# sanderslab/magellanmapper

Measured on AMD Instinct MI355X. Metric: Mvoxels/s, 2048x2048x1024 uint16 stack, 5-sigma LoG blob detection, higher is better.
Workload: dtype f16x2 MFMA (f32 accumulate) + 16-bit fixed-point intermediates; f64 re-score of every candidate

## Files before the change

magellanmapper_amd/csrc/mmx_peaks.hip:

```cpp

#include "mmx_common.h"

namespace {

constexpr int kSigmaChunk = 8;

struct peak_ctx {
    const float* base;
    int64_t sigma_stride;
    int ns, nz, ny, nx, px, plane, slot;
    float thr, eps;
    mmx_cand* out;
    uint32_t cap;
    uint32_t* count;
};

__device__ __forceinline__ void check_voxel(const peak_ctx& c, int s, int idx, float v)
{
    const int z = idx / c.plane;
    const int rem = idx - z * c.plane;
    const int y = rem / c.px;
    const int x = rem - y * c.px;
    const int nz = c.nz, ny = c.ny, nx = c.nx, px = c.px, plane = c.plane;
    const float reject = v + c.eps;
    float m = -INFINITY;
    bool border = false;
    const float* ps = c.base + (int64_t)s * c.sigma_stride;
    if (x > 0) m = fmaxf(m, ps[idx - 1]); else border = true;
    if (x + 1 < nx) m = fmaxf(m, ps[idx + 1]); else border = true;
    if (y > 0) m = fmaxf(m, ps[idx - px]); else border = true;
    if (y + 1 < ny) m = fmaxf(m, ps[idx + px]); else border = true;
    if (z > 0) m = fmaxf(m, ps[idx - plane]); else border = true;
    if (z + 1 < nz) m = fmaxf(m, ps[idx + plane]); else border = true;
    if (m > reject) return;
    for (int ds = -1; ds <= 1; ++ds) {
        const int ss = s + ds;
        if (ss < 0 || ss >= c.ns) { border = true; continue; }
        const float* pss = c.base + (int64_t)ss * c.sigma_stride;
        for (int dz = -1; dz <= 1; ++dz) {
            const int zz = z + dz;
            if (zz < 0 || zz >= nz) continue;
            for (int dy = -1; dy <= 1; ++dy) {
                const int yy = y + dy;
                if (yy < 0 || yy >= ny) continue;
                const int row = zz * plane + yy * px;
#pragma unroll
                for (int dx = -1; dx <= 1; ++dx) {
                    const int xx = x + dx;
                    if (xx < 0 || xx >= nx) continue;
                    if ((ds | dz | dy | dx) == 0) continue;
                    m = fmaxf(m, pss[row + xx]);
                }
            }
            if (m > reject) return;
        }
    }
    if (border) m = fmaxf(m, 0.0f);
    if (!(v >= m - c.eps)) return;
    const bool contested = !(v > m + c.eps) || !(v > c.thr + c.eps);
    const uint32_t pos = atomicAdd(c.count, 1u);
    if (pos < c.cap) {
        mmx_cand r;
        r.slot = c.slot;
        r.s = s;
        r.z = z;
        r.y = y;
        r.x = x;
        r.flags = contested ? MMX_CAND_CONTESTED : 0u;
        r.v = v;
        r.nbr_max = m;
        r.v64 = __longlong_as_double(0x7ff8000000000000LL);
        r.band = 0;
        c.out[pos] = r;
    }
}

__global__ void __launch_bounds__(MMX_WG)
peaks_kernel(const float* __restrict__ log, int ns, int64_t sigma_stride,
             const mmx_block* __restrict__ blocks, int64_t slot_elems, float thr, float eps,
             mmx_cand* __restrict__ out, uint32_t cap, uint32_t* __restrict__ count)
{
    const mmx_block bd = blocks[blockIdx.y];
    peak_ctx c;
    c.base = log + (int64_t)bd.slot * slot_elems;
    c.sigma_stride = sigma_stride;
    c.ns = ns; c.nz = bd.nz; c.ny = bd.ny; c.nx = bd.nx; c.px = bd.px;
    c.plane = bd.ny * bd.px; c.slot = bd.slot;
    c.thr = thr; c.eps = eps; c.out = out; c.cap = cap; c.count = count;
    const int nquads = bd.nz * c.plane / 4;
    const float lo = thr - eps;
    const int qrow = bd.px / 4;

    for (int q = blockIdx.x * MMX_WG + threadIdx.x; q < nquads; q += gridDim.x * MMX_WG) {
        const int x0 = (q % qrow) * 4;
        if (x0 >= bd.nx) continue;
        const float4* p = reinterpret_cast<const float4*>(c.base) + q;
        const int64_t sstride4 = sigma_stride / 4;
        const int lane = threadIdx.x & 63;
        const bool has_left = x0 > 0 && lane > 0;
        const bool has_right = x0 + 4 < bd.nx && lane < 63 && q + 1 < nquads;
        const bool ok1 = x0 + 1 < bd.nx, ok2 = x0 + 2 < bd.nx, ok3 = x0 + 3 < bd.nx;
        for (int s0 = 0; s0 < ns; s0 += kSigmaChunk) {
            float e0[kSigmaChunk + 2], e1[kSigmaChunk + 2], e2[kSigmaChunk + 2], e3[kSigmaChunk + 2];
#pragma unroll
            for (int k = 0; k < kSigmaChunk + 2; ++k) {
                const int s = s0 + k - 1;
                float4 v = make_float4(-INFINITY, -INFINITY, -INFINITY, -INFINITY);
                if (s >= 0 && s < ns) v = p[(int64_t)s * sstride4];
                e0[k] = v.x;
                e1[k] = ok1 ? v.y : -INFINITY;
                e2[k] = ok2 ? v.z : -INFINITY;
                e3[k] = ok3 ? v.w : -INFINITY;
            }
            unsigned hits = 0;
#pragma unroll
            for (int k = 1; k <= kSigmaChunk; ++k) {
                if (s0 + k - 1 < ns) {
                    float lft = __shfl_up(e3[k], 1);
                    float rgt = __shfl_down(e0[k], 1);
                    lft = has_left ? lft : -INFINITY;
                    rgt = has_right ? rgt : -INFINITY;
                    const float n0 = fmaxf(fmaxf(lft, e1[k]), fmaxf(e0[k - 1], e0[k + 1]));
                    const float n1 = fmaxf(fmaxf(e0[k], e2[k]), fmaxf(e1[k - 1], e1[k + 1]));
                    const float n2 = fmaxf(fmaxf(e1[k], e3[k]), fmaxf(e2[k - 1], e2[k + 1]));
                    const float n3 = fmaxf(fmaxf(e2[k], rgt), fmaxf(e3[k - 1], e3[k + 1]));
                    const unsigned sh = 4 * (k - 1);
                    hits |= (mmx_candidate(true, e0[k], lo, eps, n0) ? 1u : 0u) << sh;
                    hits |= (mmx_candidate(true, e1[k], lo, eps, n1) ? 2u : 0u) << sh;
                    hits |= (mmx_candidate(true, e2[k], lo, eps, n2) ? 4u : 0u) << sh;
                    hits |= (mmx_candidate(true, e3[k], lo, eps, n3) ? 8u : 0u) << sh;
                }
            }
            while (hits) {
                const int b = __ffs(hits) - 1;
                hits &= hits - 1;
                const int j = b & 3;
                if (x0 + j >= bd.nx) continue;
                const int s = s0 + (b >> 2);
                const int idx = 4 * q + j;
                check_voxel(c, s, idx, c.base[(int64_t)s * sigma_stride + idx]);
            }
        }
    }
}

struct sparse_ctx {
    peak_ctx c;
    const ulonglong2* ent;
    int64_t ent_sigma_stride;
    mmx_entry_geom eg;
};

__device__ __forceinline__ int64_t sparse_entry(const sparse_ctx& k, int z, int y, int x)
{
    return (int64_t)y * k.eg.per_row + mmx_entry_index(k.eg, z, x);
}

__device__ __forceinline__ float sparse_at(const sparse_ctx& k, int s, int z, int y, int x)
{
    const unsigned long long above = k.ent[(int64_t)s * k.ent_sigma_stride + sparse_entry(k, z, y, x)].y;
    if (!above) return -INFINITY;
    return k.c.base[(int64_t)s * k.c.sigma_stride + (int64_t)z * k.c.plane + y * k.c.px + x];
}

__device__ __forceinline__ void check_voxel_sparse(const sparse_ctx& k, int s, int z, int y, int x, float v)
{
    const peak_ctx& c = k.c;
    const int nz = c.nz, ny = c.ny, nx = c.nx;
    const float reject = v + c.eps;
    const float band_lo = v - c.eps;
    float m = -INFINITY;
    bool border = false;
    unsigned long long band = 0;
    unsigned band_hi = 0;
    for (int ds = -1; ds <= 1; ++ds) {
        const int ss = s + ds;
        if (ss < 0 || ss >= c.ns) { border = true; continue; }
        for (int dz = -1; dz <= 1; ++dz) {
            const int zz = z + dz;
            if (zz < 0 || zz >= nz) { border = true; continue; }
            for (int dy = -1; dy <= 1; ++dy) {
                const int yy = y + dy;
                if (yy < 0 || yy >= ny) { border = true; continue; }
                const ulonglong2* er = k.ent + (int64_t)ss * k.ent_sigma_stride;
                const float* row = c.base + (int64_t)ss * c.sigma_stride + (int64_t)zz * c.plane + yy * c.px;
#pragma unroll
                for (int dx = -1; dx <= 1; ++dx) {
                    const int xx = x + dx;
                    if (xx < 0 || xx >= nx) { border = true; continue; }
                    if ((ds | dz | dy | dx) == 0) continue;
                    if (er[sparse_entry(k, zz, yy, xx)].y) {
                        const float u = row[xx];
                        m = fmaxf(m, u);
                        if (u >= band_lo) {
                            int j = (((ds + 1) * 3 + (dz + 1)) * 3 + (dy + 1)) * 3 + (dx + 1);
                            j -= j > 40;
                            if (j < 64) band |= 1ull << j;
                            else band_hi |= 1u << (j - 64);
                        }
                    }
                }
            }
            if (m > reject) return;
        }
    }
    if (border) m = fmaxf(m, 0.0f);
    if (!(v >= m - c.eps)) return;
    const bool contested = !(v > m + c.eps) || !(v > c.thr + c.eps);
    const uint32_t pos = atomicAdd(c.count, 1u);
    if (pos < c.cap) {
        mmx_cand r;
        r.slot = c.slot;
        r.s = s;
        r.z = z;
        r.y = y;
        r.x = x;
        r.flags = (contested ? MMX_CAND_CONTESTED : 0u) | MMX_CAND_BAND | (band_hi << 16);
        r.v = v;
        r.nbr_max = m;
        r.v64 = __longlong_as_double(0x7ff8000000000000LL);
        r.band = band;
        c.out[pos] = r;
    }
}

__global__ void __launch_bounds__(MMX_WG)
peaks_sparse_kernel(const float* __restrict__ log, const ulonglong2* __restrict__ entries,
                    int ns, int64_t sigma_stride, const mmx_block* __restrict__ blocks, int64_t slot_elems,
                    float thr, float eps, mmx_cand* __restrict__ out, uint32_t cap,
                    uint32_t* __restrict__ count, int quads)
{
    const mmx_block bd = blocks[blockIdx.y];
    sparse_ctx k;
    peak_ctx& c = k.c;
    c.base = log + (int64_t)bd.slot * slot_elems;
    c.sigma_stride = sigma_stride;
    c.ns = ns; c.nz = bd.nz; c.ny = bd.ny; c.nx = bd.nx; c.px = bd.px;
    c.plane = bd.ny * bd.px; c.slot = bd.slot;
    c.thr = thr; c.eps = eps; c.out = out; c.cap = cap; c.count = count;
    k.eg = mmx_entry_geom_make(quads ? MMX_MASK_QUADS : MMX_MASK_ROWS, bd.nz, bd.nx, bd.px);
    k.ent = entries + mmx_entry_base(bd.slot, slot_elems);
    k.ent_sigma_stride = sigma_stride >> 5;
    const int64_t per_sigma = (int64_t)bd.ny * k.eg.per_row;
    const int64_t total = per_sigma * ns;
    constexpr int kQ = 1024;
    __shared__ unsigned long long q[kQ];
    __shared__ int qn;
    auto test_bit = [&](int64_t i, int b) __attribute__((always_inline)) {
        const int s = (int)(i / per_sigma);
        const int64_t r = i - (int64_t)s * per_sigma;
        const int y = (int)(r / k.eg.per_row);
        const int w = (int)(r - (int64_t)y * k.eg.per_row);
        int z, x;
        mmx_entry_voxel(k.eg, w, b, &z, &x);
        if (x >= bd.nx || z >= bd.nz) return;
        const float v = c.base[(int64_t)s * sigma_stride + (int64_t)z * c.plane + y * bd.px + x];
        const float n0 = z > 0 ? sparse_at(k, s, z - 1, y, x) : -INFINITY;
        const float n1 = z + 1 < bd.nz ? sparse_at(k, s, z + 1, y, x) : -INFINITY;
        const float n2 = s > 0 ? sparse_at(k, s - 1, z, y, x) : -INFINITY;
        const float n3 = s + 1 < ns ? sparse_at(k, s + 1, z, y, x) : -INFINITY;
        if (fmaxf(fmaxf(n0, n1), fmaxf(n2, n3)) > v + eps) return;
        check_voxel_sparse(k, s, z, y, x, v);
    };
    if (threadIdx.x == 0) qn = 0;
    for (int j = threadIdx.x; j < kQ; j += MMX_WG) q[j] = ~0ull;
    __syncthreads();
    constexpr int kW = 8;
    const int64_t stride = (int64_t)gridDim.x * MMX_WG * kW;
    const int64_t rounds = (total + stride - 1) / stride;
    for (int64_t rd = 0; rd < rounds; ++rd) {
        const int64_t i0 = rd * stride + (int64_t)blockIdx.x * MMX_WG * kW + threadIdx.x;
        unsigned long long mw[kW];
#pragma unroll
        for (int u = 0; u < kW; ++u) {
            const int64_t i = i0 + (int64_t)u * MMX_WG;
            mw[u] = 0;
            if (i < total) {
                const int s = (int)(i / per_sigma);
                mw[u] = k.ent[(int64_t)s * k.ent_sigma_stride + (i - (int64_t)s * per_sigma)].x;
            }
        }
#pragma unroll
        for (int u = 0; u < kW; ++u) {
            unsigned long long m = mw[u];
            if (!m) continue;
            const int64_t i = i0 + (int64_t)u * MMX_WG;
            const int cnt = __popcll(m);
            const int at = atomicAdd(&qn, cnt);
            if (at + cnt <= kQ) {
                int j = at;
                while (m) {
                    const int b = __ffsll((long long)m) - 1;
                    m &= m - 1;
                    q[j++] = ((unsigned long long)i << 6) | (unsigned long long)b;
                }
            } else {
                while (m) {
                    const int b = __ffsll((long long)m) - 1;
                    m &= m - 1;
                    test_bit(i, b);
                }
            }
        }
        __syncthreads();
        const int nq = qn < kQ ? qn : kQ;
        for (int j = threadIdx.x; j < nq; j += MMX_WG) {
            const unsigned long long e = q[j];
            if (e != ~0ull) test_bit((int64_t)(e >> 6), (int)(e & 63));
        }
        __syncthreads();
        if (threadIdx.x == 0) qn = 0;
        for (int j = threadIdx.x; j < nq; j += MMX_WG) q[j] = ~0ull;
        __syncthreads();
    }
}

}

int mmx_launch_peaks_sparse(const float* d_log, const unsigned long long* d_mask, int n_sigma,
                            int64_t sigma_stride, const mmx_block* d_blocks, int n_blocks, int max_vox,
                            int64_t slot_elems, float thr, float eps, mmx_cand* d_cands, uint32_t cap,
                            uint32_t* d_count, int quads, hipStream_t stream)
{
    int64_t words = ((int64_t)max_vox / 64 + 1024) * n_sigma;
    int gx = (int)((words + MMX_WG * 8 - 1) / (MMX_WG * 8));
    if (gx > 8192) gx = 8192;
    if (gx < 1) gx = 1;
    dim3 grid(gx, n_blocks);
    hipLaunchKernelGGL(peaks_sparse_kernel, grid, dim3(MMX_WG), 0, stream, d_log,
                       reinterpret_cast<const ulonglong2*>(d_mask), n_sigma, sigma_stride,
                       d_blocks, slot_elems, thr, eps, d_cands, cap, d_count, quads);
    return hipGetLastError() == hipSuccess ? MMX_OK : MMX_ERR_HIP;
}

int mmx_launch_peaks(const float* d_log, int n_sigma, int64_t sigma_stride, const mmx_block* d_blocks,
                     int n_blocks, int max_vox, int64_t slot_elems, float thr, float eps,
                     mmx_cand* d_cands, uint32_t cap, uint32_t* d_count, hipStream_t stream)
{
    int gx = (max_vox / 4 + MMX_WG - 1) / MMX_WG;
    if (gx > 8192) gx = 8192;
    if (gx < 1) gx = 1;
    dim3 grid(gx, n_blocks);
    hipLaunchKernelGGL(peaks_kernel, grid, dim3(MMX_WG), 0, stream, d_log, n_sigma, sigma_stride,
                       d_blocks, slot_elems, thr, eps, d_cands, cap, d_count);
    return hipGetLastError() == hipSuccess ? MMX_OK : MMX_ERR_HIP;
}
```

magellanmapper_amd/csrc/mmx_rescore.hip:

```cpp

#include <algorithm>
#include <type_traits>

#include "mmx_common.h"

#define MMX_MAX_SIGMAS 64

struct mmx_rescore_params {
    int32_t radius[MMX_MAX_SIGMAS];
    double norm[MMX_MAX_SIGMAS];
    int32_t strip;
    int32_t n_blocks;
};

namespace {

template <typename InT> struct in_scale;
template <> struct in_scale<uint8_t>  { static __device__ double get(uint8_t v)  { return (double)v * (1.0 / 255.0); } };
template <> struct in_scale<uint16_t> { static __device__ double get(uint16_t v) { return (double)v * (1.0 / 65535.0); } };
template <> struct in_scale<float>    { static __device__ double get(float v)    { return (double)v; } };
template <> struct in_scale<double>   { static __device__ double get(double v)   { return v; } };

template <typename StoreT>
__device__ __forceinline__ double corr_at(const double* vals, int st, int R, const double* w)
{
    double acc = vals[R * st] * w[0];
    for (int k = R; k >= 1; --k) acc += (vals[(R - k) * st] + vals[(R + k) * st]) * w[k];
    return (double)(StoreT)acc;
}

#ifndef MMX_RESCORE_BATCH
#define MMX_RESCORE_BATCH 8
#endif
constexpr int kB = MMX_RESCORE_BATCH;

template <typename InT, typename StoreT>
__global__ void __launch_bounds__(MMX_WG)
rescore_kernel(const InT* __restrict__ vol, int64_t sz, int64_t sy, int64_t sx,
               const mmx_block* __restrict__ blocks, mmx_cand* __restrict__ pts, uint32_t cap,
               const uint32_t* __restrict__ count, const double* __restrict__ w0_tab,
               const double* __restrict__ w2_tab, mmx_rescore_params prm)
{
    extern __shared__ double smem[];
    uint32_t n = cap;
    if (count) { const uint32_t c = *count; n = c < cap ? c : cap; }
    for (uint64_t idx64 = blockIdx.x; idx64 < n; idx64 += gridDim.x) {
    const uint32_t idx = (uint32_t)idx64;
    const mmx_cand ptv = pts[idx];
    mmx_cand pt;
    pt.slot = __builtin_amdgcn_readfirstlane(ptv.slot);
    pt.s = __builtin_amdgcn_readfirstlane(ptv.s);
    pt.z = __builtin_amdgcn_readfirstlane(ptv.z);
    pt.y = __builtin_amdgcn_readfirstlane(ptv.y);
    pt.x = __builtin_amdgcn_readfirstlane(ptv.x);
    if (pt.slot < 0 || pt.slot >= prm.n_blocks || pt.s < 0 || pt.s >= MMX_MAX_SIGMAS) continue;
    const mmx_block bd = blocks[pt.slot];
    const int R = prm.radius[pt.s];
    const int N = 2 * R + 1;
    const int SW = prm.strip < N ? prm.strip : N;
    const double* w0 = w0_tab + (int64_t)pt.s * (MMX_MAX_RADIUS_GENERIC + 1);
    const double* w2 = w2_tab + (int64_t)pt.s * (MMX_MAX_RADIUS_GENERIC + 1);
    const InT* in = vol + bd.src_off;

    double* zp0 = smem;
    double* zp2 = zp0 + (size_t)N * SW;
    double* yp = zp2 + (size_t)N * SW;
    int64_t* zr = (int64_t*)(yp + 3 * (size_t)N);

    __syncthreads();
    for (int k = threadIdx.x; k < N; k += MMX_WG) zr[k] = (int64_t)mmx_reflect(pt.z + k - R, bd.nz) * sz;
    __syncthreads();
    for (int dx0 = 0; dx0 < N; dx0 += SW) {
        const int sw = (N - dx0) < SW ? (N - dx0) : SW;
        for (int e = threadIdx.x; e < N * sw; e += MMX_WG) {
            const int dyi = e / sw;
            const int dxi = e - dyi * sw;
            const int yy = mmx_reflect(pt.y + dyi - R, bd.ny);
            const int xx = mmx_reflect(pt.x + dx0 + dxi - R, bd.nx);
            const InT* col = in + (int64_t)yy * sy + (int64_t)xx * sx;
            const double c = in_scale<InT>::get(col[zr[R]]);
            double a0 = c * w0[0];
            double a2 = c * w2[0];
            int k = R;
            auto batch = [&](auto nb) __attribute__((always_inline)) {
                constexpr int B = decltype(nb)::value;
                for (; k >= B; k -= B) {
                    InT lo[B], hi[B];
#pragma unroll
                    for (int j = 0; j < B; ++j) {
                        lo[j] = col[zr[R - (k - j)]];
                        hi[j] = col[zr[R + (k - j)]];
                    }
#pragma unroll
                    for (int j = 0; j < B; ++j) {
                        const double p = in_scale<InT>::get(lo[j]) + in_scale<InT>::get(hi[j]);
                        a0 += p * w0[k - j];
                        a2 += p * w2[k - j];
                    }
                }
            };
            batch(std::integral_constant<int, kB>{});
            batch(std::integral_constant<int, 4>{});
            batch(std::integral_constant<int, 2>{});
            batch(std::integral_constant<int, 1>{});
            zp0[dyi * SW + dxi] = (double)(StoreT)a0;
            zp2[dyi * SW + dxi] = (double)(StoreT)a2;
        }
        __syncthreads();
        for (int t = threadIdx.x; t < 3 * sw; t += MMX_WG) {
            const int term = t / sw;
            const int dxi = t - term * sw;
            const double* src = (term == 0 ? zp2 : zp0) + dxi;
            yp[term * N + dx0 + dxi] = corr_at<StoreT>(src, SW, R, term == 1 ? w2 : w0);
        }
        __syncthreads();
    }
    if (threadIdx.x < 3)
        zp0[threadIdx.x] = corr_at<StoreT>(yp + threadIdx.x * N, 1, R, threadIdx.x == 2 ? w2 : w0);
    __syncthreads();
    if (threadIdx.x == 0) {
        const StoreT t0 = (StoreT)zp0[0];
        const StoreT t1 = (StoreT)zp0[1];
        const StoreT t2 = (StoreT)zp0[2];
        StoreT sum = t0;
        sum += t1;
        sum += t2;
        const StoreT cube = (-sum) * (StoreT)prm.norm[pt.s];
        pts[idx].v64 = (double)cube;
    }
    }
}

template <typename InT, typename StoreT>
int launch(const mmx_volume* vol, const mmx_block* d_blocks, mmx_cand* d_pts, uint32_t cap,
           const uint32_t* d_count, const double* d_w0, const double* d_w2,
           const mmx_rescore_params& prm, size_t lds, hipStream_t s)
{
    const uint32_t gx = cap < 8192u ? cap : 8192u;
    hipLaunchKernelGGL((rescore_kernel<InT, StoreT>), dim3(gx), dim3(MMX_WG), lds, s,
                       (const InT*)vol->d_data, vol->stride_z, vol->stride_y, vol->stride_x, d_blocks,
                       d_pts, cap, d_count, d_w0, d_w2, prm);
    return hipGetLastError() == hipSuccess ? MMX_OK : MMX_ERR_HIP;
}

}

namespace {
__global__ void __launch_bounds__(MMX_WG)
expand_probes_kernel(mmx_cand* __restrict__ tab, uint32_t cap, uint32_t* __restrict__ count,
                     const uint32_t* __restrict__ n_cands, const mmx_block* __restrict__ blocks, int n_blocks, int ns)
{
    const uint32_t n = *n_cands < cap ? *n_cands : cap;
    for (uint64_t i = (uint64_t)blockIdx.x * MMX_WG + threadIdx.x; i < n; i += (uint64_t)gridDim.x * MMX_WG) {
        const mmx_cand c = tab[i];
        if (!(c.flags & MMX_CAND_CONTESTED) || c.slot < 0 || c.slot >= n_blocks) continue;
        const mmx_block bd = blocks[c.slot];
        const bool banded = (c.flags & MMX_CAND_BAND) != 0;
        int j = 0;
        for (int ds = -1; ds <= 1; ++ds)
            for (int dz = -1; dz <= 1; ++dz)
                for (int dy = -1; dy <= 1; ++dy)
                    for (int dx = -1; dx <= 1; ++dx) {
                        if ((ds | dz | dy | dx) == 0) continue;
                        const int bit = j++;
                        const int ss = c.s + ds, zz = c.z + dz, yy = c.y + dy, xx = c.x + dx;
                        if (ss < 0 || ss >= ns || zz < 0 || zz >= bd.nz || yy < 0 || yy >= bd.ny || xx < 0 || xx >= bd.nx)
                            continue;
                        if (banded && !(bit < 64 ? (c.band >> bit) & 1ull : (c.flags >> (16 + bit - 64)) & 1u)) continue;
                        const uint32_t pos = atomicAdd(count, 1u);
                        if (pos < cap) {
                            mmx_cand r;
                            r.slot = c.slot; r.s = ss; r.z = zz; r.y = yy; r.x = xx;
                            r.flags = MMX_CAND_PROBE;
                            r.v = 0.f; r.nbr_max = 0.f;
                            r.v64 = __longlong_as_double(0x7ff8000000000000LL);
                            r.band = i;
                            tab[pos] = r;
                        }
                    }
    }
}
}

extern "C" int mmx_expand_probes(mmx_cand* d_cands, uint32_t cap, uint32_t* d_count, uint32_t* d_n_cands,
                                 const mmx_block* d_blocks, int n_blocks, int n_sigma, void* stream)
{
    if (!d_cands || !d_count || !d_n_cands || !d_blocks || n_blocks < 1 || n_sigma < 1) return MMX_ERR_ARG;
    hipStream_t s = (hipStream_t)stream;
    if (hipMemcpyAsync(d_n_cands, d_count, sizeof(uint32_t), hipMemcpyDeviceToDevice, s) != hipSuccess) return MMX_ERR_HIP;
    if (cap == 0) return MMX_OK;
    mmx_timed_scope ts(MMX_K_RESCORE, s);
    const uint32_t gx = std::min<uint32_t>(1024u, (cap + MMX_WG - 1) / MMX_WG);
    hipLaunchKernelGGL(expand_probes_kernel, dim3(gx), dim3(MMX_WG), 0, s, d_cands, cap, d_count, d_n_cands, d_blocks,
                       n_blocks, n_sigma);
    return hipGetLastError() == hipSuccess ? MMX_OK : MMX_ERR_HIP;
}

extern "C" int mmx_rescore_f64(const mmx_volume* vol, const mmx_block* d_blocks, int n_blocks,
                               mmx_cand* d_pts, uint32_t cap, const uint32_t* d_count,
                               const double* d_w0, const double* d_w2, const int32_t* h_radius,
                               const double* h_norm, int n_sigma, int store_f32, void* stream)
{
    if (!vol || !vol->d_data || !d_blocks || !d_pts || !d_w0 || !d_w2 || !h_radius || !h_norm)
        return MMX_ERR_ARG;
    if (n_sigma < 1 || n_sigma > MMX_MAX_SIGMAS || n_blocks < 1) return MMX_ERR_ARG;
    if (cap == 0) return MMX_OK;
    mmx_rescore_params prm;
    int rmax = 0;
    for (int i = 0; i < MMX_MAX_SIGMAS; ++i) { prm.radius[i] = 0; prm.norm[i] = 0.0; }
    for (int i = 0; i < n_sigma; ++i) {
        if (h_radius[i] < 0 || h_radius[i] > MMX_MAX_RADIUS_GENERIC) return MMX_ERR_UNSUPPORTED;
        prm.radius[i] = h_radius[i];
        prm.norm[i] = h_norm[i];
        if (h_radius[i] > rmax) rmax = h_radius[i];
    }
    prm.n_blocks = n_blocks;
    const int N = 2 * rmax + 1;
    const size_t budget = 60 * 1024;
    const size_t fixed = (size_t)3 * N * sizeof(double) + (size_t)N * sizeof(int64_t) + 16;
    int strip = (int)((budget - fixed) / ((size_t)2 * N * sizeof(double)));
    if (strip < 1) return MMX_ERR_UNSUPPORTED;
    if (strip > N) strip = N;
    prm.strip = strip;
    const size_t lds = (size_t)2 * N * strip * sizeof(double) + fixed;
    hipStream_t s = (hipStream_t)stream;
    const bool f32s = store_f32 != 0;
    mmx_timed_scope ts(MMX_K_RESCORE, s);
    switch (vol->dtype) {
        case MMX_U8:  return launch<uint8_t, double>(vol, d_blocks, d_pts, cap, d_count, d_w0, d_w2, prm, lds, s);
        case MMX_U16: return launch<uint16_t, double>(vol, d_blocks, d_pts, cap, d_count, d_w0, d_w2, prm, lds, s);
        case MMX_F32: return f32s ? launch<float, float>(vol, d_blocks, d_pts, cap, d_count, d_w0, d_w2, prm, lds, s)
                                  : launch<float, double>(vol, d_blocks, d_pts, cap, d_count, d_w0, d_w2, prm, lds, s);
        case MMX_F64: return launch<double, double>(vol, d_blocks, d_pts, cap, d_count, d_w0, d_w2, prm, lds, s);
        default: return MMX_ERR_ARG;
    }
}
```

Before: 44090.

## Warp-cooperative 3x3x3 peak check with two-stage queue and multi-column rescore

```diff
diff --git a/magellanmapper_amd/csrc/mmx_peaks.hip b/magellanmapper_amd/csrc/mmx_peaks.hip
--- a/magellanmapper_amd/csrc/mmx_peaks.hip
+++ b/magellanmapper_amd/csrc/mmx_peaks.hip
@@ -163,47 +163,51 @@
     return k.c.base[(int64_t)s * k.c.sigma_stride + (int64_t)z * k.c.plane + y * k.c.px + x];
 }
 
-__device__ __forceinline__ void check_voxel_sparse(const sparse_ctx& k, int s, int z, int y, int x, float v)
+__device__ __forceinline__ void check_voxel_sparse_group(const sparse_ctx& k, int s, int z, int y, int x, int l)
 {
     const peak_ctx& c = k.c;
     const int nz = c.nz, ny = c.ny, nx = c.nx;
-    const float reject = v + c.eps;
+    const int ds = l / 9 - 1, dz = (l / 3) % 3 - 1, dy = l % 3 - 1;
+    const int ss = s + ds, zz = z + dz, yy = y + dy;
+    const bool row_ok = l < 27 && ss >= 0 && ss < c.ns && zz >= 0 && zz < nz && yy >= 0 && yy < ny;
+    const int sc = min(max(ss, 0), c.ns - 1), zc = min(max(zz, 0), nz - 1), yc = min(max(yy, 0), ny - 1);
+    const int xl = max(x - 1, 0), xr = min(x + 1, nx - 1);
+    const float* ctr = c.base + (int64_t)s * c.sigma_stride + (int64_t)z * c.plane + y * c.px + x;
+    const ulonglong2* er = k.ent + (int64_t)sc * k.ent_sigma_stride + (int64_t)yc * k.eg.per_row;
+    const int el = mmx_entry_index(k.eg, zc, xl), em = mmx_entry_index(k.eg, zc, x), er_i = mmx_entry_index(k.eg, zc, xr);
+    const float v = *ctr;
+    const unsigned long long al = er[el].y;
+    const unsigned long long ar = er[er_i].y;
+    const unsigned long long am = em == el ? al : ar;
+    const float* row = c.base + (int64_t)sc * c.sigma_stride + (int64_t)zc * c.plane + yc * c.px;
+    const bool ok0 = row_ok && x > 0 && al != 0;
+    const bool ok1 = row_ok && l != 13 && am != 0;
+    const bool ok2 = row_ok && x + 1 < nx && ar != 0;
+    const float r0 = *(ok0 ? row + x - 1 : ctr);
+    const float r1 = *(ok1 ? row + x : ctr);
+    const float r2 = *(ok2 ? row + x + 1 : ctr);
+    const float u0 = ok0 ? r0 : -INFINITY, u1 = ok1 ? r1 : -INFINITY, u2 = ok2 ? r2 : -INFINITY;
+    float m = fmaxf(fmaxf(u0, u1), u2);
     const float band_lo = v - c.eps;
-    float m = -INFINITY;
-    bool border = false;
-    unsigned long long band = 0;
-    unsigned band_hi = 0;
-    for (int ds = -1; ds <= 1; ++ds) {
-        const int ss = s + ds;
-        if (ss < 0 || ss >= c.ns) { border = true; continue; }
-        for (int dz = -1; dz <= 1; ++dz) {
-            const int zz = z + dz;
-            if (zz < 0 || zz >= nz) { border = true; continue; }
-            for (int dy = -1; dy <= 1; ++dy) {
-                const int yy = y + dy;
-                if (yy < 0 || yy >= ny) { border = true; continue; }
-                const ulonglong2* er = k.ent + (int64_t)ss * k.ent_sigma_stride;
-                const float* row = c.base + (int64_t)ss * c.sigma_stride + (int64_t)zz * c.plane + yy * c.px;
-#pragma unroll
-                for (int dx = -1; dx <= 1; ++dx) {
-                    const int xx = x + dx;
-                    if (xx < 0 || xx >= nx) { border = true; continue; }
-                    if ((ds | dz | dy | dx) == 0) continue;
-                    if (er[sparse_entry(k, zz, yy, xx)].y) {
-                        const float u = row[xx];
-                        m = fmaxf(m, u);
-                        if (u >= band_lo) {
-                            int j = (((ds + 1) * 3 + (dz + 1)) * 3 + (dy + 1)) * 3 + (dx + 1);
-                            j -= j > 40;
-                            if (j < 64) band |= 1ull << j;
-                            else band_hi |= 1u << (j - 64);
-                        }
-                    }
-                }
-            }
-            if (m > reject) return;
-        }
-    }
+    unsigned b_lo = 0, b_mid = 0, b_hi = 0;
+    auto mark = [&](bool in, int j) __attribute__((always_inline)) {
+        j -= j > 40;
+        const unsigned bit = in ? 1u << (j & 31) : 0u;
+        if (j < 32) b_lo |= bit; else if (j < 64) b_mid |= bit; else b_hi |= bit;
+    };
+    mark(u0 >= band_lo, 3 * l);
+    mark(u1 >= band_lo, 3 * l + 1);
+    mark(u2 >= band_lo, 3 * l + 2);
+#pragma unroll
+    for (int d = 16; d >= 1; d >>= 1) {
+        m = fmaxf(m, __shfl_xor(m, d, 32));
+        b_lo |= (unsigned)__shfl_xor((int)b_lo, d, 32);
+        b_mid |= (unsigned)__shfl_xor((int)b_mid, d, 32);
+        b_hi |= (unsigned)__shfl_xor((int)b_hi, d, 32);
+    }
+    if (l != 0) return;
+    if (m > v + c.eps) return;
+    const bool border = s == 0 || s + 1 == c.ns || z == 0 || z + 1 == nz || y == 0 || y + 1 == ny || x == 0 || x + 1 == nx;
     if (border) m = fmaxf(m, 0.0f);
     if (!(v >= m - c.eps)) return;
     const bool contested = !(v > m + c.eps) || !(v > c.thr + c.eps);
@@ -215,11 +219,11 @@
         r.z = z;
         r.y = y;
         r.x = x;
-        r.flags = (contested ? MMX_CAND_CONTESTED : 0u) | MMX_CAND_BAND | (band_hi << 16);
+        r.flags = (contested ? MMX_CAND_CONTESTED : 0u) | MMX_CAND_BAND | (b_hi << 16);
         r.v = v;
         r.nbr_max = m;
         r.v64 = __longlong_as_double(0x7ff8000000000000LL);
-        r.band = band;
+        r.band = ((unsigned long long)b_mid << 32) | b_lo;
         c.out[pos] = r;
     }
 }
@@ -244,26 +248,55 @@
     const int64_t per_sigma = (int64_t)bd.ny * k.eg.per_row;
     const int64_t total = per_sigma * ns;
     constexpr int kQ = 1024;
+    constexpr int kQ2 = 512;
     __shared__ unsigned long long q[kQ];
-    __shared__ int qn;
-    auto test_bit = [&](int64_t i, int b) __attribute__((always_inline)) {
-        const int s = (int)(i / per_sigma);
-        const int64_t r = i - (int64_t)s * per_sigma;
-        const int y = (int)(r / k.eg.per_row);
-        const int w = (int)(r - (int64_t)y * k.eg.per_row);
-        int z, x;
-        mmx_entry_voxel(k.eg, w, b, &z, &x);
-        if (x >= bd.nx || z >= bd.nz) return;
-        const float v = c.base[(int64_t)s * sigma_stride + (int64_t)z * c.plane + y * bd.px + x];
-        const float n0 = z > 0 ? sparse_at(k, s, z - 1, y, x) : -INFINITY;
-        const float n1 = z + 1 < bd.nz ? sparse_at(k, s, z + 1, y, x) : -INFINITY;
-        const float n2 = s > 0 ? sparse_at(k, s - 1, z, y, x) : -INFINITY;
-        const float n3 = s + 1 < ns ? sparse_at(k, s + 1, z, y, x) : -INFINITY;
-        if (fmaxf(fmaxf(n0, n1), fmaxf(n2, n3)) > v + eps) return;
-        check_voxel_sparse(k, s, z, y, x, v);
+    __shared__ unsigned long long q2[kQ2];
+    __shared__ int qn, q2n;
+    auto voxel_of = [&](unsigned long long e, int* s, int* z, int* y, int* x) __attribute__((always_inline)) -> bool {
+        const int64_t i = (int64_t)(e >> 6);
+        *s = (int)(i / per_sigma);
+        const int64_t r = i - (int64_t)*s * per_sigma;
+        *y = (int)(r / k.eg.per_row);
+        const int w = (int)(r - (int64_t)*y * k.eg.per_row);
+        mmx_entry_voxel(k.eg, w, (int)(e & 63), z, x);
+        return *x < bd.nx && *z < bd.nz;
     };
-    if (threadIdx.x == 0) qn = 0;
-    for (int j = threadIdx.x; j < kQ; j += MMX_WG) q[j] = ~0ull;
+    auto pre_check = [&](unsigned long long e) __attribute__((always_inline)) -> bool {
+        int s, z, y, x;
+        const bool real = voxel_of(e, &s, &z, &y, &x);
+        z = min(z, bd.nz - 1);
+        x = min(x, bd.nx - 1);
+        const float* ctr = c.base + (int64_t)s * sigma_stride + (int64_t)z * c.plane + y * bd.px + x;
+        const int zd = max(z - 1, 0), zu = min(z + 1, bd.nz - 1), sd = max(s - 1, 0), su = min(s + 1, ns - 1);
+        const ulonglong2* ey = k.ent + (int64_t)y * k.eg.per_row;
+        const int64_t es = (int64_t)s * k.ent_sigma_stride;
+        const int ec = mmx_entry_index(k.eg, z, x);
+        const float v = *ctr;
+        const unsigned long long a0 = ey[es + mmx_entry_index(k.eg, zd, x)].y;
+        const unsigned long long a1 = ey[es + mmx_entry_index(k.eg, zu, x)].y;
+        const unsigned long long a2 = ey[(int64_t)sd * k.ent_sigma_stride + ec].y;
+        const unsigned long long a3 = ey[(int64_t)su * k.ent_sigma_stride + ec].y;
+        const bool ok0 = z > 0 && a0 != 0, ok1 = z + 1 < bd.nz && a1 != 0, ok2 = s > 0 && a2 != 0, ok3 = s + 1 < ns && a3 != 0;
+        const float r0 = *(ok0 ? ctr - c.plane : ctr);
+        const float r1 = *(ok1 ? ctr + c.plane : ctr);
+        const float r2 = *(ok2 ? ctr - sigma_stride : ctr);
+        const float r3 = *(ok3 ? ctr + sigma_stride : ctr);
+        const float n0 = ok0 ? r0 : -INFINITY, n1 = ok1 ? r1 : -INFINITY, n2 = ok2 ? r2 : -INFINITY, n3 = ok3 ? r3 : -INFINITY;
+        return real && !(fmaxf(fmaxf(n0, n1), fmaxf(n2, n3)) > v + eps);
+    };
+    auto full_test = [&]() __attribute__((always_inline)) {
+        __syncthreads();
+        const int n2 = q2n;
+        const int l = threadIdx.x & 31;
+        for (int t = threadIdx.x >> 5; t < n2; t += MMX_WG / 32) {
+            int s, z, y, x;
+            voxel_of(q2[t], &s, &z, &y, &x);
+            check_voxel_sparse_group(k, s, z, y, x, l);
+        }
+        __syncthreads();
+        if (threadIdx.x == 0) q2n = 0;
+    };
+    if (threadIdx.x == 0) { qn = 0; q2n = 0; }
     __syncthreads();
     constexpr int kW = 8;
     const int64_t stride = (int64_t)gridDim.x * MMX_WG * kW;
@@ -280,38 +313,41 @@
                 mw[u] = k.ent[(int64_t)s * k.ent_sigma_stride + (i - (int64_t)s * per_sigma)].x;
             }
         }
-#pragma unroll
-        for (int u = 0; u < kW; ++u) {
-            unsigned long long m = mw[u];
-            if (!m) continue;
-            const int64_t i = i0 + (int64_t)u * MMX_WG;
-            const int cnt = __popcll(m);
-            const int at = atomicAdd(&qn, cnt);
-            if (at + cnt <= kQ) {
-                int j = at;
-                while (m) {
+        for (;;) {
+            bool left = false;
+#pragma unroll
+            for (int u = 0; u < kW; ++u) {
+                unsigned long long m = mw[u];
+                if (!m || left) { left = left || m != 0; continue; }
+                const int64_t i = i0 + (int64_t)u * MMX_WG;
+                const int cnt = __popcll(m);
+                const int at = atomicAdd(&qn, cnt);
+                int fit = kQ - at;
+                fit = fit < 0 ? 0 : fit < cnt ? fit : cnt;
+                for (int j = at; j < at + fit; ++j) {
                     const int b = __ffsll((long long)m) - 1;
                     m &= m - 1;
-                    q[j++] = ((unsigned long long)i << 6) | (unsigned long long)b;
+                    q[j] = ((unsigned long long)i << 6) | (unsigned long long)b;
                 }
-            } else {
-                while (m) {
-                    const int b = __ffsll((long long)m) - 1;
-                    m &= m - 1;
-                    test_bit(i, b);
+                mw[u] = m;
+                left = m != 0;
+            }
+            __syncthreads();
+            const int nq = qn < kQ ? qn : kQ;
+            for (int j0 = 0; j0 < nq; j0 += MMX_WG) {
+                const int j = j0 + threadIdx.x;
+                const unsigned long long e = j < nq ? q[j] : 0;
+                if (j < nq && pre_check(e)) q2[atomicAdd(&q2n, 1)] = e;
+                if (j0 + MMX_WG < nq) {
+                    __syncthreads();
+                    if (q2n > kQ2 - MMX_WG) full_test();
+                    __syncthreads();
                 }
             }
-        }
-        __syncthreads();
-        const int nq = qn < kQ ? qn : kQ;
-        for (int j = threadIdx.x; j < nq; j += MMX_WG) {
-            const unsigned long long e = q[j];
-            if (e != ~0ull) test_bit((int64_t)(e >> 6), (int)(e & 63));
-        }
-        __syncthreads();
-        if (threadIdx.x == 0) qn = 0;
-        for (int j = threadIdx.x; j < nq; j += MMX_WG) q[j] = ~0ull;
-        __syncthreads();
+            full_test();
+            if (threadIdx.x == 0) qn = 0;
+            if (!__syncthreads_or(left)) break;
+        }
     }
 }
 
diff --git a/magellanmapper_amd/csrc/mmx_rescore.hip b/magellanmapper_amd/csrc/mmx_rescore.hip
--- a/magellanmapper_amd/csrc/mmx_rescore.hip
+++ b/magellanmapper_amd/csrc/mmx_rescore.hip
@@ -29,10 +29,109 @@
     return (double)(StoreT)acc;
 }
 
-#ifndef MMX_RESCORE_BATCH
-#define MMX_RESCORE_BATCH 8
-#endif
-constexpr int kB = MMX_RESCORE_BATCH;
+constexpr int kLoadRegs = 16;
+constexpr int kMaxCols = 4;
+template <typename InT, int NC>
+struct z_cfg {
+    static constexpr int raw = kLoadRegs / (2 * NC);
+    static constexpr int TB = raw >= 8 ? 8 : raw >= 4 ? 4 : raw >= 2 ? 2 : 1;
+};
+__host__ __device__ __forceinline__ int rescore_col_class(int ncols)
+{
+    const int cols = (ncols + MMX_WG - 1) / MMX_WG;
+    const int passes = (cols + kMaxCols - 1) / kMaxCols;
+    const int per = (cols + passes - 1) / passes;
+    return per <= 1 ? 1 : per <= 2 ? 2 : 4;
+}
+
+template <typename T> struct off_type { using type = T; };
+
+template <typename InT, typename StoreT, int NC, bool INTERIOR, typename OffT>
+__device__ __forceinline__ void z_phase(const InT* __restrict__ in, int nyb, int nxb, int pz, int py, int px0, int R, int N,
+                                        int SW, int sw, int64_t sz, int64_t sy, int64_t sx,
+                                        const int64_t* __restrict__ zr, const double* __restrict__ w0,
+                                        const double* __restrict__ w2, double* __restrict__ zp0, double* __restrict__ zp2)
+{
+    constexpr int TB = z_cfg<InT, NC>::TB;
+    const int ncols = N * sw;
+    auto zoff = [&](int j) __attribute__((always_inline)) -> int64_t {
+        if constexpr (INTERIOR) return (int64_t)(pz + j - R) * sz;
+        else return zr[j];
+    };
+    constexpr bool kBytes = sizeof(OffT) == 4;
+    auto ld = [&](OffT o, int64_t z) __attribute__((always_inline)) -> InT {
+        if constexpr (kBytes) return *reinterpret_cast<const InT*>(reinterpret_cast<const char*>(in + z) + o);
+        else return in[o + z];
+    };
+    for (int base = 0; base < ncols; base += MMX_WG * NC) {
+        OffT off[NC];
+        int at[NC];
+#pragma unroll
+        for (int c = 0; c < NC; ++c) {
+            const int e = base + c * MMX_WG + (int)threadIdx.x;
+            const int ec = e < ncols ? e : ncols - 1;
+            const int dyi = ec / sw;
+            const int dxi = ec - dyi * sw;
+            const int yy = mmx_reflect(py + dyi - R, nyb);
+            const int xx = mmx_reflect(px0 + dxi - R, nxb);
+            off[c] = (OffT)(((int64_t)yy * sy + (int64_t)xx * sx) * (kBytes ? (int64_t)sizeof(InT) : 1));
+            at[c] = e < ncols ? dyi * SW + dxi : -1;
+        }
+        double a0[NC], a2[NC];
+        {
+            const int64_t zc = zoff(R);
+            InT ctr[NC];
+#pragma unroll
+            for (int c = 0; c < NC; ++c) ctr[c] = ld(off[c], zc);
+#pragma unroll
+            for (int c = 0; c < NC; ++c) {
+                const double cv = in_scale<InT>::get(ctr[c]);
+                a0[c] = cv * w0[0];
+                a2[c] = cv * w2[0];
+            }
+        }
+        int k = R;
+        auto batch = [&](auto nb) __attribute__((always_inline)) {
+            constexpr int B = decltype(nb)::value;
+            for (; k >= B; k -= B) {
+                InT lo[NC][B], hi[NC][B];
+                if constexpr (kBytes) {
+#pragma unroll
+                    for (int c = 0; c < NC; ++c) asm volatile("" : "+v"(off[c]));
+                }
+#pragma unroll
+                for (int j = 0; j < B; ++j) {
+                    const int64_t zl = zoff(R - (k - j)), zh = zoff(R + (k - j));
+#pragma unroll
+                    for (int c = 0; c < NC; ++c) {
+                        lo[c][j] = ld(off[c], zl);
+                        hi[c][j] = ld(off[c], zh);
+                    }
+                }
+#pragma unroll
+                for (int c = 0; c < NC; ++c) {
+#pragma unroll
+                    for (int j = 0; j < B; ++j) {
+                        const double p = in_scale<InT>::get(lo[c][j]) + in_scale<InT>::get(hi[c][j]);
+                        a0[c] += p * w0[k - j];
+                        a2[c] += p * w2[k - j];
+                    }
+                }
+            }
+        };
+        batch(std::integral_constant<int, TB>{});
+        if constexpr (TB > 4) batch(std::integral_constant<int, 4>{});
+        if constexpr (TB > 2) batch(std::integral_constant<int, 2>{});
+        if constexpr (TB > 1) batch(std::integral_constant<int, 1>{});
+#pragma unroll
+        for (int c = 0; c < NC; ++c) {
+            if (at[c] >= 0) {
+                zp0[at[c]] = (double)(StoreT)a0[c];
+                zp2[at[c]] = (double)(StoreT)a2[c];
+            }
+        }
+    }
+}
 
 template <typename InT, typename StoreT>
 __global__ void __launch_bounds__(MMX_WG)
@@ -67,44 +166,32 @@
     double* yp = zp2 + (size_t)N * SW;
     int64_t* zr = (int64_t*)(yp + 3 * (size_t)N);
 
+    const bool interior = pt.z - R >= 0 && pt.z + R < bd.nz;
+    const int cls = rescore_col_class(N * SW);
+    const bool small = ((int64_t)(bd.ny - 1) * sy + (int64_t)(bd.nx - 1) * sx) * (int64_t)sizeof(InT) < (1ll << 31)
+                       && sy >= 0 && sx >= 0;
     __syncthreads();
-    for (int k = threadIdx.x; k < N; k += MMX_WG) zr[k] = (int64_t)mmx_reflect(pt.z + k - R, bd.nz) * sz;
-    __syncthreads();
+    if (!interior) {
+        for (int k = threadIdx.x; k < N; k += MMX_WG) zr[k] = (int64_t)mmx_reflect(pt.z + k - R, bd.nz) * sz;
+        __syncthreads();
+    }
     for (int dx0 = 0; dx0 < N; dx0 += SW) {
         const int sw = (N - dx0) < SW ? (N - dx0) : SW;
-        for (int e = threadIdx.x; e < N * sw; e += MMX_WG) {
-            const int dyi = e / sw;
-            const int dxi = e - dyi * sw;
-            const int yy = mmx_reflect(pt.y + dyi - R, bd.ny);
-            const int xx = mmx_reflect(pt.x + dx0 + dxi - R, bd.nx);
-            const InT* col = in + (int64_t)yy * sy + (int64_t)xx * sx;
-            const double c = in_scale<InT>::get(col[zr[R]]);
-            double a0 = c * w0[0];
-            double a2 = c * w2[0];
-            int k = R;
-            auto batch = [&](auto nb) __attribute__((always_inline)) {
-                constexpr int B = decltype(nb)::value;
-                for (; k >= B; k -= B) {
-                    InT lo[B], hi[B];
-#pragma unroll
-                    for (int j = 0; j < B; ++j) {
-                        lo[j] = col[zr[R - (k - j)]];
-                        hi[j] = col[zr[R + (k - j)]];
-                    }
-#pragma unroll
-                    for (int j = 0; j < B; ++j) {
-                        const double p = in_scale<InT>::get(lo[j]) + in_scale<InT>::get(hi[j]);
-                        a0 += p * w0[k - j];
-                        a2 += p * w2[k - j];
-                    }
-                }
-            };
-            batch(std::integral_constant<int, kB>{});
-            batch(std::integral_constant<int, 4>{});
-            batch(std::integral_constant<int, 2>{});
-            batch(std::integral_constant<int, 1>{});
-            zp0[dyi * SW + dxi] = (double)(StoreT)a0;
-            zp2[dyi * SW + dxi] = (double)(StoreT)a2;
+        auto zrun = [&](auto nc, auto ot) __attribute__((always_inline)) {
+            constexpr int NC = decltype(nc)::value;
+            using OffT = typename decltype(ot)::type;
+            if (interior)
+                z_phase<InT, StoreT, NC, true, OffT>(in, bd.ny, bd.nx, pt.z, pt.y, pt.x + dx0, R, N, SW, sw, sz, sy, sx,
+                                                     zr, w0, w2, zp0, zp2);
+            else
+                z_phase<InT, StoreT, NC, false, OffT>(in, bd.ny, bd.nx, pt.z, pt.y, pt.x + dx0, R, N, SW, sw, sz, sy, sx,
+                                                      zr, w0, w2, zp0, zp2);
+        };
+        if (!small) zrun(std::integral_constant<int, 2>{}, off_type<int64_t>{});
+        else switch (cls) {
+            case 1: zrun(std::integral_constant<int, 1>{}, off_type<uint32_t>{}); break;
+            case 2: zrun(std::integral_constant<int, 2>{}, off_type<uint32_t>{}); break;
+            default: zrun(std::integral_constant<int, 4>{}, off_type<uint32_t>{}); break;
         }
         __syncthreads();
         for (int t = threadIdx.x; t < 3 * sw; t += MMX_WG) {
```

After: 44960, median of 6. 1.02x the previous value.
